# shengyangsun/LSTC_VAD

Measured on AMD Instinct MI355X. Metric: snippets/sec training step (B=64,T=32,P=16,d=2048), higher is better.
Workload: dtype f32

## Files before the change

### include/lstc_hip.h

```cpp
#ifndef LSTC_HIP_H
#define LSTC_HIP_H

#include <stdint.h>

#ifdef __cplusplus
extern "C" {
#endif

#define LSTC_VERSION 112

enum {
    LSTC_OK = 0,
    LSTC_E_NULL = -1,
    LSTC_E_SHAPE = -2,
    LSTC_E_ALIGN = -3,
    LSTC_E_UNSUPPORTED = -4,
    LSTC_E_RANGE = -5
};

enum { LSTC_F32 = 0, LSTC_BF16 = 1, LSTC_F32X3 = 2, LSTC_BF16P = 3 };

enum {
    LSTC_EPI_BIAS = 1, LSTC_EPI_RELU = 2, LSTC_EPI_DROPOUT = 4, LSTC_EPI_RESIDUAL = 8,
    LSTC_EPI_RELU_MASK = 16, LSTC_EPI_ACCUM = 32, LSTC_EPI_OUT_F32 = 64,
// ... 20 lines not shown
    const void* A;
    const void* B;
    void*       C;
    const float* bias;
    const void*  residual;
    const void*  relu_src;
} LstcGemmDesc;

int lstc_gemm(const LstcGemmDesc* d, void* stream);

int32_t lstc_gemm_splits(int32_t dtype, int32_t K, int32_t split_k);

int64_t lstc_pack3_bytes(int64_t rows, int64_t K);
int lstc_pack3(const float* src, int64_t rows, int64_t K, int64_t ld, int32_t k_major, void* dst, void* stream);

int64_t lstc_pack1_bytes(int64_t rows, int64_t K);
int lstc_pack1(const float* src, int64_t rows, int64_t K, int64_t ld, int32_t k_major, void* dst, void* stream);
typedef struct LstcPackItem {
    const float* src; int64_t rows, K, ld; int32_t k_major; void* dst;
} LstcPackItem;
int lstc_pack1_multi(const LstcPackItem* items, int32_t count, void* stream);
int lstc_colsum_pack1(const void* packed, int64_t rows, int32_t K, float* partial, int32_t n_partial, float* out,
                      int32_t accumulate, void* stream);

typedef struct LstcAttnDesc {
    int32_t N, S, H, dk, dv;
    int32_t ldq, ldk, ldv, ldo;
    int32_t dtype;
    int32_t index_ld;
    int32_t table_rows;
    float   scale;
    float   dropout_p;
    uint64_t dropout_seed;
    const void* Q; const void* K; const void* V;
    void*  O;
    float* probs;
    const float*   table;
    const int64_t* index;
    const void* dO;
    void* dQ; void* dK; void* dV;
    float* dtable;
    int32_t dtable_chunks;
    int32_t variant;
    void* dQ_pack; void* dK_pack; void* dV_pack;
    int32_t pack_cols, dQ_col0, dK_col0, dV_col0;
    void* O_pack;
// ... 129 lines not shown
```

### lstc_vad_amd/csrc/attention.hip

```cpp
#include "attention_common.h"

#ifndef ATTN_HEAD_FAST
#define ATTN_HEAD_FAST 0
#endif
#if ATTN_HEAD_FAST
#define ATTN_CHUNK ((int)blockIdx.y)
#define ATTN_HEAD ((int)blockIdx.x)
#define ATTN_GRID(chunks, H) dim3((unsigned)(H), (unsigned)(chunks))
#else
#define ATTN_CHUNK ((int)blockIdx.x)
#define ATTN_HEAD ((int)blockIdx.y)
#define ATTN_GRID(chunks, H) dim3((unsigned)(chunks), (unsigned)(H))
#endif

namespace {
using namespace lstc_attn;

constexpr int NT = 256;


__device__ __forceinline__ void load16(const float* __restrict__ p, int k0, int kdim, bool vec, float (&f)[16]) {
    if (vec && k0 + 16 <= kdim) {
        const float4* q = reinterpret_cast<const float4*>(p + k0);
#pragma unroll
// ... 759 lines not shown

extern "C" {

int lstc_attn_fwd(const LstcAttnDesc* d, void* stream) {
    AttnParams p;
    int rc = fill_params(d, p, false);
    if (rc) return rc;
    if (p.S > 128) return attn_long_fwd_launch(d, p, (hipStream_t)stream);
    if (d->O_pack) {
        const int64_t M = (int64_t)p.N * p.S;
        if (M % 256 || (p.H * p.dv) % 64 || p.dv % 32 || M * (int64_t)(p.H * p.dv) * 2 > 0x7fffffffLL) return LSTC_E_UNSUPPORTED;
        if (!aligned16(d->O_pack)) return LSTC_E_ALIGN;
        p.Op = d->O_pack;
        p.kbo = (p.H * p.dv) / 32;
    }
    hipStream_t st = (hipStream_t)stream;
    const bool bf = d->dtype == LSTC_BF16;
    const int T = (p.S + 31) / 32;
    if (d->in_pack_cols > 0) {
        if (!d->O_pack) return LSTC_E_UNSUPPORTED;
        rc = fill_packed_inputs(d, p, false);
        if (rc) return rc;
        int npw = (int)(((int64_t)p.N * p.H) / (T == 1 ? 8192 : 1024));
        if (d->variant >= 100) npw = d->variant - 100;
        npw = npw < 1 ? 1 : (npw > 16 ? 16 : npw);
        p.n_per_wg = npw;
        dim3 grid3((p.N + npw - 1) / npw, p.H);
        return attn3_fwd_launch(p, T, (int)grid3.x, st);
    }
    if (!bf && (d->variant == 3 || (d->variant == 0 && T != 2)) && d->O && T <= 3 && p.vec_qk && p.vec_v && p.dk % 32 == 0 && p.dv % 64 == 0) {
        int npw = (int)(((int64_t)p.N * p.H) / (T == 1 ? 8192 : 1024));
        npw = npw < 1 ? 1 : (npw > 16 ? 16 : npw);
        p.n_per_wg = npw;
        return attn3f_fwd_launch(p, T, (p.N + npw - 1) / npw, st);
    }
    const size_t lds = (size_t)(32 * T) * (32 * T + 1) * sizeof(float);
    dim3 grid = ATTN_GRID(p.N, p.H);
    if ((T == 1 || T == 3 || (bf && T == 2)) && p.vec_qk && p.vec_v && (p.dk % 32) == 0 && (p.dv % 32) == 0 && (d->variant == 0 || d->variant == 2)) {
        const int SP = 32 * T;
        const size_t lds2 = ((size_t)((SP * (SP + 1) + 3) & ~3) + (size_t)4 * SP * 32) * sizeof(float);
#define LSTC_FWD2(TT, BB, WW)                                                              \
    do {                                                                                   \
        static LstcDevOnce once2;                                                          \
        const int dev2_ = once2.begin();                                                   \
        if (dev2_ >= 0) { set_lds(attn_fwd2_kernel<TT, BB, WW>, 160 * 1024); once2.end(dev2_); } \
        hipLaunchKernelGGL((attn_fwd2_kernel<TT, BB, WW>), grid, 64 * WW, lds2, st, p);    \
    } while (0)
        if (!bf) { if (T == 1) LSTC_FWD2(1, false, 4); else LSTC_FWD2(3, false, 8); }
        else if (T == 1) LSTC_FWD2(1, true, 4); else if (T == 2) LSTC_FWD2(2, true, 4); else LSTC_FWD2(3, true, 8);
// ... 49 lines not shown
    p.n_per_wg = npw;
    const int chunks_ = (p.N + npw - 1) / npw;
    dim3 grid = ATTN_GRID(chunks_, p.H);
    if (p.table_partials && chunks_ != d->dtable_chunks) return LSTC_E_SHAPE;
    const bool v2 = T <= 3 && p.vec_qk && p.vec_v && (p.dk % 32) == 0 && (p.dv % 32) == 0 && d->variant != 1;
    if (d->dQ_pack || d->dK_pack || d->dV_pack) {
        const int64_t M = (int64_t)p.N * p.S;
        if (!(d->dQ_pack && d->dK_pack && d->dV_pack) || (!v2 && d->in_pack_cols <= 0) || M % 256 || (p.H * p.dk) % 64 || (p.H * p.dv) % 64 ||
            M * (int64_t)(p.H * (p.dk > p.dv ? p.dk : p.dv)) * 2 > 0x7fffffffLL) return LSTC_E_UNSUPPORTED;
        if (!aligned16(d->dQ_pack) || !aligned16(d->dK_pack) || !aligned16(d->dV_pack)) return LSTC_E_ALIGN;
        p.dQp = d->dQ_pack; p.dKp = d->dK_pack; p.dVp = d->dV_pack;
        p.kbq = p.kbk = (p.H * p.dk) / 32;
        p.kbv = (p.H * p.dv) / 32;
        if (d->pack_cols > 0) {
            if (d->pack_cols % 64 || d->dQ_col0 % 32 || d->dK_col0 % 32 || d->dV_col0 % 32 || d->dQ_col0 < 0 || d->dK_col0 < 0 || d->dV_col0 < 0 ||
                d->dQ_col0 + p.H * p.dk > d->pack_cols || d->dK_col0 + p.H * p.dk > d->pack_cols || d->dV_col0 + p.H * p.dv > d->pack_cols ||
                M * (int64_t)d->pack_cols * 2 > 0x7fffffffLL) return LSTC_E_SHAPE;
            p.kbq = p.kbk = p.kbv = d->pack_cols / 32;
            p.tq0 = d->dQ_col0 / 32; p.tk0 = d->dK_col0 / 32; p.tv0 = d->dV_col0 / 32;
        }
    }
    if (d->in_pack_cols > 0) {
        if (!p.dQp) return LSTC_E_UNSUPPORTED;
        return attn3_bwd_launch(p, T, chunks_, st);
    }
    if (v2) {
        const int SP = 32 * T, NW = T == 3 ? 8 : 4;
        const size_t lds2 = ((size_t)((2 * SP * (SP + 1) + 3) & ~3) + (size_t)4 * SP * 32 + (size_t)NW * p.table_rows) * sizeof(float);
        if (lds2 <= 160 * 1024) {
#define LSTC_BWD2(TT, BB, WW)                                                              \
    do {                                                                                   \
        static LstcDevOnce once2;                                                          \
        const int dev2_ = once2.begin();                                                   \
        if (dev2_ >= 0) { set_lds(attn_bwd2_kernel<TT, BB, WW>, 160 * 1024); once2.end(dev2_); } \
        hipLaunchKernelGGL((attn_bwd2_kernel<TT, BB, WW>), grid, 64 * WW, lds2, st, p);    \
    } while (0)
            if (T == 1) { if (bf) LSTC_BWD2(1, true, 4); else LSTC_BWD2(1, false, 4); }
            else if (T == 2) { if (bf) LSTC_BWD2(2, true, 4); else LSTC_BWD2(2, false, 4); }
            else { if (bf) LSTC_BWD2(3, true, 8); else LSTC_BWD2(3, false, 8); }
#undef LSTC_BWD2
            return lstc_launch_status();
        }
    }
    if (p.dQp) return LSTC_E_UNSUPPORTED;
#define LSTC_BWD(TT)                                                         \
    do {                                                                     \
// ... 721 lines not shown
```

### lstc_vad_amd/csrc/attention_common.h

```cpp
#pragma once
#include "lstc_common.h"

namespace lstc_attn {

struct AttnParams {
    const float *Q, *K, *V;
    float* O;
    float* probs;
    const float* table;
    const int64_t* index;
    const float* dO;
    float *dQ, *dK, *dV;
    float* dtable;
    int N, S, H, dk, dv, ldq, ldk, ldv, ldo, index_ld, table_rows;
    float scale;
    DropKey dkey;
    int has_drop;
    int vec_qk, vec_v;
    int n_per_wg;
    int table_partials;
    void *dQp, *dKp, *dVp;
    int kbq, kbk, kbv;
    int tq0, tk0, tv0;
    void* Op;
    int kbo;
    const __bf16 *Qi, *Ki, *Vi, *dOi;
    int kiq, kik, kiv, kido;
    int iq0, ik0, iv0, ido0;
    int pld;
};

typedef __bf16 attn_h8 __attribute__((ext_vector_type(8)));
typedef float attn_f2 __attribute__((ext_vector_type(2)));
typedef __bf16 attn_h2 __attribute__((ext_vector_type(2)));

__attribute__((visibility("hidden"))) int attn3_fwd_launch(const AttnParams& p, int T, int chunks, hipStream_t st);
__attribute__((visibility("hidden"))) int attn3_bwd_launch(const AttnParams& p, int T, int chunks, hipStream_t st);
__attribute__((visibility("hidden"))) int attn3f_fwd_launch(const AttnParams& p, int T, int chunks, hipStream_t st);
__attribute__((visibility("hidden"))) int attn_long_fwd_launch(const LstcAttnDesc* d, AttnParams& p, hipStream_t st);
__attribute__((visibility("hidden"))) int attn_long_bwd_launch(const LstcAttnDesc* d, AttnParams& p, hipStream_t st);

}
```

### lstc_vad_amd/csrc/attention_pk.hip

```cpp
#include "attention_common.h"

namespace {
using namespace lstc_attn;

typedef short a3_s4 __attribute__((ext_vector_type(4)));
typedef short a3_s8 __attribute__((ext_vector_type(8)));
typedef uint32_t a3_u4 __attribute__((ext_vector_type(4)));
typedef float a3_f4 __attribute__((ext_vector_type(4)));
typedef a3_s4 __attribute__((address_space(3))) * a3_lds4;

#ifndef A3_DMA_MOD
#define A3_DMA_MOD ""
#endif
__device__ __forceinline__ void a3_dma(const __bf16* tile, uint32_t voff, uint32_t lds_bytes) {
    const uint32_t lb = __builtin_amdgcn_readfirstlane(lds_bytes);
    asm volatile("s_mov_b32 m0, %2\n\ts_nop 0\n\tglobal_load_lds_dwordx4 %0, %1" A3_DMA_MOD :: "v"(voff), "s"(tile), "s"(lb) : "memory");
}
__device__ __forceinline__ uint32_t a3_row_off(uint32_t g, uint32_t kb, uint32_t lane) {
    return ((g >> 7) * kb * 4096u + (g & 127u) * 32u) * 2u + (lane & 3u) * 16u;
}
__device__ __forceinline__ attn_h8 a3_tr(const char* p0, const char* p1) {
    const a3_s4 lo = __builtin_amdgcn_ds_read_tr16_b64_v4i16((a3_lds4)p0);
    const a3_s4 hi = __builtin_amdgcn_ds_read_tr16_b64_v4i16((a3_lds4)p1);
    a3_s8 f;
// ... 8 lines not shown
    for (int g = 0; g < 4; ++g)
#pragma unroll
        for (int k = 0; k < 2; ++k) {
            attn_f2 f;
            f[0] = o[4 * g + 2 * k] * scale;
            f[1] = o[4 * g + 2 * k + 1] * scale;
            d[g][k] = __builtin_bit_cast(uint32_t, __builtin_convertvector(f, attn_h2));
        }
#pragma unroll
    for (int k = 0; k < 2; ++k) {
        const auto x = __builtin_amdgcn_permlane32_swap(d[0][k], d[2][k], false, false);
        d[0][k] = x[0]; d[2][k] = x[1];
        const auto y = __builtin_amdgcn_permlane32_swap(d[1][k], d[3][k], false, false);
        d[1][k] = y[0]; d[3][k] = y[1];
    }
    const uint32_t base = rowb + tile * 8192u;
    const a3_u4 ca = {d[0][0], d[0][1], d[2][0], d[2][1]}, cb = {d[1][0], d[1][1], d[3][0], d[3][1]};
    __builtin_amdgcn_raw_buffer_store_b128(ca, rs, valid ? base + ((((uint32_t)(2 * h2)) ^ key) << 4) : 0xFFFFFFFFu, 0, 0);
    __builtin_amdgcn_raw_buffer_store_b128(cb, rs, valid ? base + ((((uint32_t)(2 * h2 + 1)) ^ key) << 4) : 0xFFFFFFFFu, 0, 0);
}
#define A3_LDS_BARRIER() do { asm volatile("" ::: "memory"); __builtin_amdgcn_s_waitcnt(0xC07F); __builtin_amdgcn_s_barrier(); asm volatile("" ::: "memory"); } while (0)
#define A3_WAIT_VM(N) __builtin_amdgcn_s_waitcnt(((N) & 15) | (7 << 4) | (15 << 8) | (((N) >> 4) << 14))

struct A3Unit { const __bf16 *b0, *b1; uint32_t kb0, kb1; };

template <int T, int NB, typename UnitOf, typename Extra>
__device__ __forceinline__ void a3_producer(int n_begin, int n_end, int U, int S, UnitOf unit_of, Extra extra) {
    constexpr int SP = 32 * T, HALF = SP * 64, SLOT = 2 * HALF, P = 4 * T;
    static_assert(P * (NB - 2) <= 63, "vmcnt is a 6-bit counter");
    const int lane = threadIdx.x & 63;
    const int total = (n_end - n_begin) * U;
    int is_n = n_begin, is_u = 0, is_slot = 0, issued = 0;
    auto issue_next = [&]() {
        if (issued >= total) return;
        const A3Unit un = unit_of(is_u);
        const uint32_t lb = (uint32_t)(is_slot * SLOT);
#pragma unroll
        for (int pc = 0; pc < 2 * T; ++pc) {
            const uint32_t g = (uint32_t)is_n * (uint32_t)S + (uint32_t)min(16 * pc + (lane >> 2), S - 1);
            a3_dma(un.b0, a3_row_off(g, un.kb0, lane), lb + pc * 1024);
            a3_dma(un.b1, a3_row_off(g, un.kb1, lane), lb + HALF + pc * 1024);
        }
        ++issued;
        if (++is_u == U) { is_u = 0; ++is_n; }
        if (++is_slot == NB) is_slot = 0;
    };
#pragma unroll 1
    for (int k = 0; k < NB - 1; ++k) issue_next();
    int g = 0;
#pragma unroll 1
    for (int n = n_begin; n < n_end; ++n)
#pragma unroll 1
        for (int u = 0; u < U; ++u) {
            const int rem = min(NB - 2, total - 1 - g);
            if (rem >= NB - 2) A3_WAIT_VM(P * (NB - 2));
            else if (NB > 3 && rem == NB - 3) A3_WAIT_VM(P * (NB > 3 ? NB - 3 : 0));
            else if (NB > 4 && rem == NB - 4) A3_WAIT_VM(P * (NB > 4 ? NB - 4 : 0));
            else A3_WAIT_VM(0);
            __builtin_amdgcn_s_barrier();
            issue_next();
            const int nx = extra(u);
            for (int x = 0; x < nx; ++x) __builtin_amdgcn_s_barrier();
            ++g;
        }
}

template <int T, int NB>
__global__ void __launch_bounds__(64 * (T + 1)) attn_fwd3_kernel(const AttnParams p) {
    const DropKey dkn = drop_key_now(p.dkey);
    constexpr int SP = 32 * T, HALF = SP * 64, SLOT = 2 * HALF;
    extern __shared__ __attribute__((aligned(16))) float sm[];
    const char* ring = reinterpret_cast<const char*>(sm);
    const int h = (int)(blockIdx.x % (unsigned)p.H), chunk = (int)(blockIdx.x / (unsigned)p.H), S = p.S;
    const int lane = threadIdx.x & 63, wave = __builtin_amdgcn_readfirstlane(threadIdx.x >> 6);
    const int l31 = lane & 31, h2 = lane >> 5;
    const int n_begin = chunk * p.n_per_wg, n_end = min(p.N, n_begin + p.n_per_wg);
    const int nq = p.dk >> 5, nvp = p.dv >> 6, U = nq + nvp;
    if (wave == T) {
        const int tq = p.iq0 + ((h * p.dk) >> 5), tk = p.ik0 + ((h * p.dk) >> 5), tv = p.iv0 + ((h * p.dv) >> 5);
        a3_producer<T, NB>(n_begin, n_end, U, S,
            [&](int u) -> A3Unit {
                A3Unit un;
                if (u < nq) {
                    un.b0 = p.Qi + (size_t)(tq + u) * 4096; un.kb0 = (uint32_t)p.kiq;
                    un.b1 = p.Ki + (size_t)(tk + u) * 4096; un.kb1 = (uint32_t)p.kik;
                } else {
                    un.b0 = p.Vi + (size_t)(tv + 2 * (u - nq)) * 4096; un.kb0 = un.kb1 = (uint32_t)p.kiv;
                    un.b1 = un.b0 + 4096;
                }
                return un;
            },
            [](int) { return 0; });
        return;
    }
    const int i = 32 * wave + l31;
    const bool has_bias = p.index_ld > 0 && S > 1;
    const __amdgpu_buffer_rsrc_t r_index = __builtin_amdgcn_make_buffer_rsrc(const_cast<int64_t*>(p.index), 0,
        has_bias ? (S - 1) * p.index_ld * 8 : 0, 0x00020000);
    const __amdgpu_buffer_rsrc_t r_table = __builtin_amdgcn_make_buffer_rsrc(const_cast<float*>(p.table), 0,
        has_bias ? (p.table_rows > 0 ? p.table_rows * p.H * 4 : 0x7fffffff) : 0, 0x00020000);
    float biasr[T][16];
#pragma unroll
    for (int t = 0; t < T; ++t)
#pragma unroll
        for (int r = 0; r < 16; ++r) {
            const int j = 32 * t + 8 * (r >> 2) + 4 * h2 + (r & 3);
            const bool pair = i >= 1 && j >= 1 && i < S && j < S;
            const uint32_t ix = __builtin_amdgcn_raw_buffer_load_b32(r_index, pair ? (uint32_t)((i - 1) * p.index_ld + (j - 1)) * 8u : 0xFFFFFFFFu, 0, 0);
            const float b = __builtin_bit_cast(float, __builtin_amdgcn_raw_buffer_load_b32(r_table, ((ix * (uint32_t)p.H + (uint32_t)h) * 4u) | (pair ? 0u : 0xFFFFFFFFu), 0, 0));
            biasr[t][r] = b + (j < S ? 0.f : -INFINITY);
        }
    const __amdgpu_buffer_rsrc_t r_Op = __builtin_amdgcn_make_buffer_rsrc(p.Op, 0, (int)0x7fffffff, 0x00020000);
    const int q4 = (lane >> 2) & 3, p4 = lane & 3, gg = (lane >> 4) & 1;
    int cslot = 0;
    floatx16 acc[T];
    attn_h8 pf[T][2];
#pragma unroll 1
    for (int n = n_begin; n < n_end; ++n) {
        const uint32_t r0 = (uint32_t)n * (uint32_t)S;
        const uint32_t keyq = ((r0 + (uint32_t)i) >> 2) & 3u, keyk = ((r0 + (uint32_t)l31) >> 2) & 3u;
        const int offq0 = i * 64 + (int)(((0 + h2) ^ keyq) << 4), offq1 = i * 64 + (int)(((2 + h2) ^ keyq) << 4);
        const int offk0 = l31 * 64 + (int)(((0 + h2) ^ keyk) << 4), offk1 = l31 * 64 + (int)(((2 + h2) ^ keyk) << 4);
        int troff[2];
#pragma unroll
        for (int rd = 0; rd < 2; ++rd) {
            const uint32_t row = (uint32_t)(4 * h2 + 8 * rd + q4);
            troff[rd] = (int)(row * 64u + ((((uint32_t)(2 * gg + (p4 >> 1))) ^ (((r0 + row) >> 2) & 3u)) << 4) + 8u * (uint32_t)(p4 & 1));
        }
        const uint32_t orow = a3_row_off(r0 + (uint32_t)i, (uint32_t)p.kbo, 0);
#pragma unroll 1
        for (int u = 0; u < U; ++u) {
            A3_LDS_BARRIER();
            const char* slot = ring + cslot * SLOT;
            if (u < nq) {
                if (u == 0) {
#pragma unroll
                    for (int t = 0; t < T; ++t)
#pragma unroll
                        for (int r = 0; r < 16; ++r) acc[t][r] = 0.f;
                }
                const attn_h8 fq0 = a3_row(slot + offq0), fq1 = a3_row(slot + offq1);
#pragma unroll
                for (int t = 0; t < T; ++t) {
                    const attn_h8 fk0 = a3_row(slot + HALF + t * 2048 + offk0), fk1 = a3_row(slot + HALF + t * 2048 + offk1);
                    acc[t] = __builtin_amdgcn_mfma_f32_32x32x16_bf16(fk0, fq0, acc[t], 0, 0, 0);
                    acc[t] = __builtin_amdgcn_mfma_f32_32x32x16_bf16(fk1, fq1, acc[t], 0, 0, 0);
                }
                if (u == nq - 1) {
                    float m = -INFINITY;
#pragma unroll
                    for (int t = 0; t < T; ++t)
#pragma unroll
                        for (int r = 0; r < 16; ++r) {
                            const float x = acc[t][r] * p.scale + biasr[t][r];
                            acc[t][r] = x;
                            m = fmaxf(m, x);
                        }
                    m = fmaxf(m, __shfl_xor(m, 32, 64));
                    float sum = 0.f;
#pragma unroll
                    for (int t = 0; t < T; ++t)
#pragma unroll
                        for (int r = 0; r < 16; ++r) {
                            const float e = expf(acc[t][r] - m);
                            acc[t][r] = e;
                            sum += e;
                        }
// ... 17 lines not shown
                                float v = pv[e];
                                if (p.has_drop) v = drop_keep(flat_i + (uint32_t)(j0 + e), dkn) ? v * dkn.scale : 0.f;
                                acc[t][4 * g4 + e] = v;
                            }
                        }
#pragma unroll
                        for (int s2 = 0; s2 < 2; ++s2)
#pragma unroll
                            for (int e = 0; e < 8; ++e) pf[t][s2][e] = (__bf16)acc[t][8 * s2 + e];
                    }
                }
            } else {
                const int ct = 2 * (u - nq);
#pragma unroll
                for (int hf = 0; hf < 2; ++hf) {
                    const char* Vs = slot + hf * HALF;
                    floatx16 o[1];
#pragma unroll
                    for (int r = 0; r < 16; ++r) o[0][r] = 0.f;
#pragma unroll
                    for (int t = 0; t < T; ++t)
#pragma unroll
                        for (int s2 = 0; s2 < 2; ++s2) {
                            const attn_h8 fv = a3_tr(Vs + t * 2048 + s2 * 1024 + troff[0], Vs + t * 2048 + s2 * 1024 + troff[1]);
                            o[0] = __builtin_amdgcn_mfma_f32_32x32x16_bf16(fv, pf[t][s2], o[0], 0, 0, 0);
                        }
                    a3_store_tile(o[0], 1.f, r_Op, orow, keyq, i < S, (uint32_t)(((h * p.dv) >> 5) + ct + hf), h2);
                }
            }
            if (++cslot == NB) cslot = 0;
        }
    }
}

template <int T, int NB>
__global__ void __launch_bounds__(64 * (T + 1)) attn_bwd3_kernel(const AttnParams p) {
    const DropKey dkn = drop_key_now(p.dkey);
    constexpr int SP = 32 * T, HALF = SP * 64, SLOT = 2 * HALF;
    constexpr int ILD = 72, IMG = SP * ILD;
    extern __shared__ __attribute__((aligned(16))) float sm[];
    char* ring = reinterpret_cast<char*>(sm);
    char* img = ring + NB * SLOT;
    float* tacc = reinterpret_cast<float*>(img + IMG);
    const int h = (int)(blockIdx.x % (unsigned)p.H), chunk = (int)(blockIdx.x / (unsigned)p.H), S = p.S;
    const int lane = threadIdx.x & 63, wave = __builtin_amdgcn_readfirstlane(threadIdx.x >> 6);
    const int l31 = lane & 31, h2 = lane >> 5;
    const int n_begin = chunk * p.n_per_wg, n_end = min(p.N, n_begin + p.n_per_wg);
    const int nv = p.dv >> 5, nq2 = p.dk >> 6, nv2 = p.dv >> 6;
    const int u_c1 = nv, u_c2 = nv + nq2, u_c3 = nv + nq2 + nv2, U = nv + 2 * nq2 + nv2;
    const bool has_bias = p.index_ld > 0 && p.dtable != nullptr;
    if (has_bias)
        for (int x = threadIdx.x; x < T * p.table_rows; x += 64 * (T + 1)) tacc[x] = 0.f;
    __syncthreads();
    if (wave == T) {
        const int tq = p.iq0 + ((h * p.dk) >> 5), tk = p.ik0 + ((h * p.dk) >> 5), tv = p.iv0 + ((h * p.dv) >> 5), tdo = p.ido0 + ((h * p.dv) >> 5);
        a3_producer<T, NB>(n_begin, n_end, U, S,
            [&](int u) -> A3Unit {
                A3Unit un;
                if (u < u_c1) {
                    un.b0 = p.dOi + (size_t)(tdo + u) * 4096; un.kb0 = (uint32_t)p.kido;
                    un.b1 = p.Vi + (size_t)(tv + u) * 4096; un.kb1 = (uint32_t)p.kiv;
                } else if (u < u_c2) {
                    un.b0 = p.Ki + (size_t)(tk + 2 * (u - u_c1)) * 4096; un.kb0 = un.kb1 = (uint32_t)p.kik; un.b1 = un.b0 + 4096;
                } else if (u < u_c3) {
                    un.b0 = p.dOi + (size_t)(tdo + 2 * (u - u_c2)) * 4096; un.kb0 = un.kb1 = (uint32_t)p.kido; un.b1 = un.b0 + 4096;
                } else {
                    un.b0 = p.Qi + (size_t)(tq + 2 * (u - u_c3)) * 4096; un.kb0 = un.kb1 = (uint32_t)p.kiq; un.b1 = un.b0 + 4096;
                }
                return un;
            },
            [&](int u) { return u == u_c1 - 1 ? 4 * T : 0; });
    } else {
    const int i = 32 * wave + l31;
    float* const tw = tacc + wave * p.table_rows;
    const __amdgpu_buffer_rsrc_t r_index = __builtin_amdgcn_make_buffer_rsrc(const_cast<int64_t*>(p.index), 0,
        (has_bias && S > 1) ? (S - 1) * p.index_ld * 8 : 0, 0x00020000);
    uint32_t idxp[T][8];
#pragma unroll
    for (int t = 0; t < T; ++t)
#pragma unroll
        for (int r2 = 0; r2 < 8; ++r2) {
            uint32_t w2 = 0;
#pragma unroll
            for (int e = 0; e < 2; ++e) {
                const int r = 2 * r2 + e;
                const int j = 32 * t + 8 * (r >> 2) + 4 * h2 + (r & 3);
                const bool pair = has_bias && i >= 1 && j >= 1 && i < S && j < S;
                const uint32_t v = __builtin_amdgcn_raw_buffer_load_b32(r_index, pair ? (uint32_t)((i - 1) * p.index_ld + (j - 1)) * 8u : 0xFFFFFFFFu, 0, 0)
                                   | (pair ? 0u : 0xFFFFu);
                w2 |= (v & 0xFFFFu) << (16 * e);
            }
            idxp[t][r2] = w2;
        }
    const __amdgpu_buffer_rsrc_t r_dQ = __builtin_amdgcn_make_buffer_rsrc(p.dQp, 0, (int)0x7fffffff, 0x00020000);
    const __amdgpu_buffer_rsrc_t r_dK = __builtin_amdgcn_make_buffer_rsrc(p.dKp, 0, (int)0x7fffffff, 0x00020000);
    const __amdgpu_buffer_rsrc_t r_dV = __builtin_amdgcn_make_buffer_rsrc(p.dVp, 0, (int)0x7fffffff, 0x00020000);
    const int q4 = (lane >> 2) & 3, p4 = lane & 3, gg = (lane >> 4) & 1;
    char* const img_w = img + i * ILD + 8 * h2;
    const char* const img_r = img + (8 * h2 + q4) * ILD + 32 * gg + 8 * p4;
    int cslot = 0;
    floatx16 acc[T];
    float prr[T][16];
    attn_h8 dAf[T][2], PdTf[T][2], dATf[T][2];
    float dsum[T][16];
#pragma unroll
    for (int t = 0; t < T; ++t)
#pragma unroll
        for (int r = 0; r < 16; ++r) dsum[t][r] = 0.f;
#pragma unroll 1
    for (int n = n_begin; n < n_end; ++n) {
        const uint32_t r0 = (uint32_t)n * (uint32_t)S;
        const uint32_t keyq = ((r0 + (uint32_t)i) >> 2) & 3u, keyk = ((r0 + (uint32_t)l31) >> 2) & 3u;
        const int offq0 = i * 64 + (int)(((0 + h2) ^ keyq) << 4), offq1 = i * 64 + (int)(((2 + h2) ^ keyq) << 4);
        const int offk0 = l31 * 64 + (int)(((0 + h2) ^ keyk) << 4), offk1 = l31 * 64 + (int)(((2 + h2) ^ keyk) << 4);
        int troff[2], trnat[2];
#pragma unroll
        for (int rd = 0; rd < 2; ++rd) {
            const uint32_t row = (uint32_t)(4 * h2 + 8 * rd + q4), rown = (uint32_t)(8 * h2 + 4 * rd + q4);
            troff[rd] = (int)(row * 64u + ((((uint32_t)(2 * gg + (p4 >> 1))) ^ (((r0 + row) >> 2) & 3u)) << 4) + 8u * (uint32_t)(p4 & 1));
            trnat[rd] = (int)(rown * 64u + ((((uint32_t)(2 * gg + (p4 >> 1))) ^ (((r0 + rown) >> 2) & 3u)) << 4) + 8u * (uint32_t)(p4 & 1));
        }
#pragma unroll 1
        for (int u = 0; u < U; ++u) {
            A3_LDS_BARRIER();
            const char* slot = ring + cslot * SLOT;
            if (u < u_c1) {
                if (u == 0) {
                    const float* pr_item = p.probs + ((size_t)n * p.H + h) * S * p.pld;
#pragma unroll
                    for (int t = 0; t < T; ++t)
#pragma unroll
                        for (int g4 = 0; g4 < 4; ++g4) {
                            const int j0 = 32 * t + 8 * g4 + 4 * h2;
                            const bool ok = i < S && j0 < p.pld;
                            const a3_u4 v = *reinterpret_cast<const a3_u4*>(pr_item + (ok ? i * p.pld + j0 : 0));
                            const uint32_t mask = ok ? 0xFFFFFFFFu : 0u;
#pragma unroll
                            for (int e = 0; e < 4; ++e) prr[t][4 * g4 + e] = __builtin_bit_cast(float, v[e] & mask);
                        }
#pragma unroll
                    for (int t = 0; t < T; ++t)
#pragma unroll
                        for (int r = 0; r < 16; ++r) acc[t][r] = 0.f;
                }
                const attn_h8 fo0 = a3_row(slot + offq0), fo1 = a3_row(slot + offq1);
#pragma unroll
                for (int t = 0; t < T; ++t) {
                    const attn_h8 fv0 = a3_row(slot + HALF + t * 2048 + offk0), fv1 = a3_row(slot + HALF + t * 2048 + offk1);
                    acc[t] = __builtin_amdgcn_mfma_f32_32x32x16_bf16(fv0, fo0, acc[t], 0, 0, 0);
                    acc[t] = __builtin_amdgcn_mfma_f32_32x32x16_bf16(fv1, fo1, acc[t], 0, 0, 0);
                }
                if (u == u_c1 - 1) {
                    typedef __bf16 h4v __attribute__((ext_vector_type(4)));
                    const uint32_t flat_i = ((uint32_t)n * p.H + h) * (uint32_t)(S * S) + (uint32_t)(i * S);
                    float rs = 0.f;
                    h4v pdp[T][4];
#pragma unroll
                    for (int t = 0; t < T; ++t)
#pragma unroll
                        for (int g4 = 0; g4 < 4; ++g4) {
#pragma unroll
                            for (int e = 0; e < 4; ++e) {
                                const int r = 4 * g4 + e;
                                const int j = 32 * t + 8 * g4 + 4 * h2 + e;
                                const float keep = p.has_drop ? (drop_keep(flat_i + (uint32_t)j, dkn) ? dkn.scale : 0.f) : 1.f;
                                const float dpk = acc[t][r] * keep;
                                rs += dpk * prr[t][r];
                                acc[t][r] = dpk;
                                pdp[t][g4][e] = (__bf16)(prr[t][r] * keep);
                            }
                        }
// ... 39 lines not shown
#pragma unroll
                            for (int ti = 0; ti < T; ++ti)
#pragma unroll
                                for (int s2 = 0; s2 < 2; ++s2)
                                    dATf[ti][s2] = a3_tr(img_r + (32 * ti + 16 * s2) * ILD, img_r + (32 * ti + 16 * s2 + 4) * ILD);
                        }
                        A3_LDS_BARRIER();
                    }
                }
            } else {
                const int ph = u < u_c2 ? 0 : (u < u_c3 ? 1 : 2);
                const int ct = 2 * (u - (ph == 0 ? u_c1 : (ph == 1 ? u_c2 : u_c3)));
#pragma unroll
                for (int hf = 0; hf < 2; ++hf) {
                    const char* Bs = slot + hf * HALF;
                    floatx16 o[1];
#pragma unroll
                    for (int r = 0; r < 16; ++r) o[0][r] = 0.f;
                    if (ph == 0) {
#pragma unroll
                        for (int t = 0; t < T; ++t)
#pragma unroll
                            for (int s2 = 0; s2 < 2; ++s2) {
                                const attn_h8 fb = a3_tr(Bs + t * 2048 + s2 * 1024 + troff[0], Bs + t * 2048 + s2 * 1024 + troff[1]);
                                o[0] = __builtin_amdgcn_mfma_f32_32x32x16_bf16(fb, dAf[t][s2], o[0], 0, 0, 0);
                            }
                        a3_store_tile(o[0], p.scale, r_dQ, a3_row_off(r0 + (uint32_t)i, (uint32_t)p.kbq, 0), keyq, i < S, (uint32_t)(p.tq0 + ((h * p.dk) >> 5) + ct + hf), h2);
                    } else if (ph == 1) {
#pragma unroll
                        for (int t = 0; t < T; ++t)
#pragma unroll
                            for (int s2 = 0; s2 < 2; ++s2) {
                                const attn_h8 fb = a3_tr(Bs + t * 2048 + s2 * 1024 + trnat[0], Bs + t * 2048 + s2 * 1024 + trnat[1]);
                                o[0] = __builtin_amdgcn_mfma_f32_32x32x16_bf16(fb, PdTf[t][s2], o[0], 0, 0, 0);
                            }
                        a3_store_tile(o[0], 1.f, r_dV, a3_row_off(r0 + (uint32_t)i, (uint32_t)p.kbv, 0), keyq, i < S, (uint32_t)(p.tv0 + ((h * p.dv) >> 5) + ct + hf), h2);
                    } else {
#pragma unroll
                        for (int t = 0; t < T; ++t)
#pragma unroll
                            for (int s2 = 0; s2 < 2; ++s2) {
                                const attn_h8 fb = a3_tr(Bs + t * 2048 + s2 * 1024 + trnat[0], Bs + t * 2048 + s2 * 1024 + trnat[1]);
                                o[0] = __builtin_amdgcn_mfma_f32_32x32x16_bf16(fb, dATf[t][s2], o[0], 0, 0, 0);
                            }
                        a3_store_tile(o[0], p.scale, r_dK, a3_row_off(r0 + (uint32_t)i, (uint32_t)p.kbk, 0), keyq, i < S, (uint32_t)(p.tk0 + ((h * p.dk) >> 5) + ct + hf), h2);
                    }
                }
            }
            if (++cslot == NB) cslot = 0;
        }
    }
    if (has_bias) {
#pragma unroll
        for (int t = 0; t < T; ++t)
#pragma unroll
            for (int r = 0; r < 16; ++r) {
                const uint32_t ix = (idxp[t][r >> 1] >> (16 * (r & 1))) & 0xFFFFu;
                if (ix != 0xFFFFu) atomicAdd(&tw[ix], dsum[t][r]);
            }
    }
    }
    if (has_bias) {
        __syncthreads();
        for (int x = threadIdx.x; x < p.table_rows; x += 64 * (T + 1)) {
            float v = tacc[x];
#pragma unroll
            for (int w = 1; w < T; ++w) v += tacc[w * p.table_rows + x];
            if (p.table_partials) p.dtable[((size_t)chunk * p.table_rows + x) * p.H + h] = v;
            else atomicAdd(&p.dtable[(size_t)x * p.H + h], v);
        }
    }
}

struct A3UnitF { const float *b0, *b1; uint32_t ld0, ld1; };

// ... 190 lines not shown
                        for (int g4 = 0; g4 < 4; ++g4) {
                            a3_f4 v;
#pragma unroll
                            for (int e = 0; e < 4; ++e) v[e] = o[4 * g4 + e];
                            *reinterpret_cast<a3_f4*>(o_row + 32 * (ct + hf) + 8 * g4 + 4 * h2) = v;
                        }
                    }
                }
            }
            if (++cslot == NB) cslot = 0;
        }
    }
}

template <typename Kern>
void set_lds(Kern k, size_t lds) {
    (void)hipFuncSetAttribute(reinterpret_cast<const void*>(k), hipFuncAttributeMaxDynamicSharedMemorySize, (int)lds);
}

}

namespace lstc_attn {

int attn3_fwd_launch(const AttnParams& p, int T, int chunks, hipStream_t st) {
#define LSTC_FWD3(TT, NBB)                                                                 \
    do {                                                                                   \
        static LstcDevOnce once3;                                                          \
        const int dev3_ = once3.begin();                                                   \
        if (dev3_ >= 0) { set_lds(attn_fwd3_kernel<TT, NBB>, 160 * 1024); once3.end(dev3_); } \
        hipLaunchKernelGGL((attn_fwd3_kernel<TT, NBB>), dim3((unsigned)chunks * (unsigned)p.H), 64 * (TT + 1), \
                           (size_t)NBB * 2 * (32 * TT) * 64, st, p);                       \
    } while (0)
    if (T == 1) LSTC_FWD3(1, 6); else if (T == 2) LSTC_FWD3(2, 9); else if (T == 3) LSTC_FWD3(3, 6); else return LSTC_E_RANGE;
#undef LSTC_FWD3
    return lstc_launch_status();
}

int attn3f_fwd_launch(const AttnParams& p, int T, int chunks, hipStream_t st) {
#define LSTC_FWD3F(TT, NBB)                                                                \
    do {                                                                                   \
        static LstcDevOnce once3;                                                          \
        const int dev3_ = once3.begin();                                                   \
        if (dev3_ >= 0) { set_lds(attn_fwd3f_kernel<TT, NBB>, 160 * 1024); once3.end(dev3_); } \
        hipLaunchKernelGGL((attn_fwd3f_kernel<TT, NBB>), dim3((unsigned)chunks * (unsigned)p.H), 64 * (TT + 1), \
                           (size_t)NBB * 2 * (32 * TT) * 128, st, p);                      \
    } while (0)
    if (T == 1) LSTC_FWD3F(1, 3); else if (T == 2) LSTC_FWD3F(2, 3); else if (T == 3) LSTC_FWD3F(3, 3); else return LSTC_E_RANGE;
#undef LSTC_FWD3F
    return lstc_launch_status();
}

int attn3_bwd_launch(const AttnParams& p, int T, int chunks, hipStream_t st) {
#define LSTC_BWD3(TT, NBB)                                                                 \
    do {                                                                                   \
        const size_t lds3 = (size_t)NBB * 2 * (32 * TT) * 64 + (size_t)(32 * TT) * 72 + (size_t)TT * p.table_rows * sizeof(float); \
        if (lds3 > 160 * 1024) return LSTC_E_RANGE;                                        \
        static LstcDevOnce once3;                                                          \
        const int dev3_ = once3.begin();                                                   \
        if (dev3_ >= 0) { set_lds(attn_bwd3_kernel<TT, NBB>, 160 * 1024); once3.end(dev3_); } \
        hipLaunchKernelGGL((attn_bwd3_kernel<TT, NBB>), dim3((unsigned)chunks * (unsigned)p.H), 64 * (TT + 1), lds3, st, p); \
    } while (0)
    if (T == 1) LSTC_BWD3(1, 9); else if (T == 2) LSTC_BWD3(2, 8); else if (T == 3) LSTC_BWD3(3, 5); else return LSTC_E_RANGE;
#undef LSTC_BWD3
    return lstc_launch_status();
}

}
```

Before: 22870.

## Size attention LDS ring to actual sequence rows and pick depth at runtime

The packed bf16 attention forward and backward kernels now size their LDS staging ring to the real sequence length, S rounded up to 4 rows, instead of the full 32*T padded tile. The ring depth is chosen on the host to balance pipeline depth against workgroups per CU, and launch bounds now request multiple waves per EU. The producer loads only the rows it needs, the last key/value tile maps rows with a clamped index, and the vmcnt wait becomes a runtime switch. The backward kernel also defers the index/bias gather until after the main loop to cut register pressure. The cost is extra address arithmetic, a switch-based wait, and possible reads of stale rows in partially filled tiles.

```diff
diff --git a/include/lstc_hip.h b/include/lstc_hip.h
--- a/include/lstc_hip.h
+++ b/include/lstc_hip.h
@@ -66,6 +66,8 @@
 int lstc_pack1_multi(const LstcPackItem* items, int32_t count, void* stream);
 int lstc_colsum_pack1(const void* packed, int64_t rows, int32_t K, float* partial, int32_t n_partial, float* out,
                       int32_t accumulate, void* stream);
+
+#define LSTC_ATTN_VARIANT_RING32 (1 << 30)
 
 typedef struct LstcAttnDesc {
     int32_t N, S, H, dk, dv;
diff --git a/lstc_vad_amd/csrc/attention.hip b/lstc_vad_amd/csrc/attention.hip
--- a/lstc_vad_amd/csrc/attention.hip
+++ b/lstc_vad_amd/csrc/attention.hip
@@ -805,9 +805,11 @@
         rc = fill_packed_inputs(d, p, false);
         if (rc) return rc;
         int npw = (int)(((int64_t)p.N * p.H) / (T == 1 ? 8192 : 1024));
-        if (d->variant >= 100) npw = d->variant - 100;
+        const int hook = d->variant & ~LSTC_ATTN_VARIANT_RING32;
+        if (hook >= 100) npw = hook - 100;
         npw = npw < 1 ? 1 : (npw > 16 ? 16 : npw);
         p.n_per_wg = npw;
+        p.ring_wide = (d->variant & LSTC_ATTN_VARIANT_RING32) != 0;
         dim3 grid3((p.N + npw - 1) / npw, p.H);
         return attn3_fwd_launch(p, T, (int)grid3.x, st);
     }
@@ -903,6 +905,7 @@
     }
     if (d->in_pack_cols > 0) {
         if (!p.dQp) return LSTC_E_UNSUPPORTED;
+        p.ring_wide = (d->variant & LSTC_ATTN_VARIANT_RING32) != 0;
         return attn3_bwd_launch(p, T, chunks_, st);
     }
     if (v2) {
diff --git a/lstc_vad_amd/csrc/attention_common.h b/lstc_vad_amd/csrc/attention_common.h
--- a/lstc_vad_amd/csrc/attention_common.h
+++ b/lstc_vad_amd/csrc/attention_common.h
@@ -28,6 +28,7 @@
     int kiq, kik, kiv, kido;
     int iq0, ik0, iv0, ido0;
     int pld;
+    int ring_wide, ring_rows, ring_nb;
 };
 
 typedef __bf16 attn_h8 __attribute__((ext_vector_type(8)));
diff --git a/lstc_vad_amd/csrc/attention_pk.hip b/lstc_vad_amd/csrc/attention_pk.hip
--- a/lstc_vad_amd/csrc/attention_pk.hip
+++ b/lstc_vad_amd/csrc/attention_pk.hip
@@ -1,4 +1,5 @@
 #include "attention_common.h"
+#include <cstdlib>
 
 namespace {
 using namespace lstc_attn;
@@ -54,12 +55,23 @@
 #define A3_LDS_BARRIER() do { asm volatile("" ::: "memory"); __builtin_amdgcn_s_waitcnt(0xC07F); __builtin_amdgcn_s_barrier(); asm volatile("" ::: "memory"); } while (0)
 #define A3_WAIT_VM(N) __builtin_amdgcn_s_waitcnt(((N) & 15) | (7 << 4) | (15 << 8) | (((N) >> 4) << 14))
 
+__device__ __forceinline__ void a3_wait_vm(int n) {
+    switch (n) {
+#define A3_W(N) case N: A3_WAIT_VM(N); break;
+        A3_W(2) A3_W(4) A3_W(6) A3_W(8) A3_W(10) A3_W(12) A3_W(14) A3_W(16) A3_W(18) A3_W(20) A3_W(22) A3_W(24) A3_W(26) A3_W(28) A3_W(30) A3_W(32)
+        A3_W(34) A3_W(36) A3_W(38) A3_W(40) A3_W(42) A3_W(44) A3_W(46) A3_W(48) A3_W(50) A3_W(52) A3_W(54) A3_W(56) A3_W(58) A3_W(60) A3_W(62)
+#undef A3_W
+        default: A3_WAIT_VM(0); break;
+    }
+}
+
 struct A3Unit { const __bf16 *b0, *b1; uint32_t kb0, kb1; };
 
-template <int T, int NB, typename UnitOf, typename Extra>
-__device__ __forceinline__ void a3_producer(int n_begin, int n_end, int U, int S, UnitOf unit_of, Extra extra) {
-    constexpr int SP = 32 * T, HALF = SP * 64, SLOT = 2 * HALF, P = 4 * T;
-    static_assert(P * (NB - 2) <= 63, "vmcnt is a 6-bit counter");
+__device__ __forceinline__ int a3_tile_row(int row, int SR) { return row < SR ? row : SR - 4 + (row & 3); }
+
+template <int T, typename UnitOf, typename Extra>
+__device__ __forceinline__ void a3_producer(int n_begin, int n_end, int U, int S, int SR, int NB, UnitOf unit_of, Extra extra) {
+    const int HALF = SR * 64, SLOT = 2 * HALF, PH = (SR + 15) >> 4, P = 2 * PH;
     const int lane = threadIdx.x & 63;
     const int total = (n_end - n_begin) * U;
     int is_n = n_begin, is_u = 0, is_slot = 0, issued = 0;
@@ -69,9 +81,13 @@
         const uint32_t lb = (uint32_t)(is_slot * SLOT);
 #pragma unroll
         for (int pc = 0; pc < 2 * T; ++pc) {
-            const uint32_t g = (uint32_t)is_n * (uint32_t)S + (uint32_t)min(16 * pc + (lane >> 2), S - 1);
-            a3_dma(un.b0, a3_row_off(g, un.kb0, lane), lb + pc * 1024);
-            a3_dma(un.b1, a3_row_off(g, un.kb1, lane), lb + HALF + pc * 1024);
+            if (pc >= PH) break;
+            const int row = 16 * pc + (lane >> 2);
+            if (row < SR) {
+                const uint32_t g = (uint32_t)is_n * (uint32_t)S + (uint32_t)min(row, S - 1);
+                a3_dma(un.b0, a3_row_off(g, un.kb0, lane), lb + pc * 1024);
+                a3_dma(un.b1, a3_row_off(g, un.kb1, lane), lb + HALF + pc * 1024);
+            }
         }
         ++issued;
         if (++is_u == U) { is_u = 0; ++is_n; }
@@ -84,11 +100,7 @@
     for (int n = n_begin; n < n_end; ++n)
 #pragma unroll 1
         for (int u = 0; u < U; ++u) {
-            const int rem = min(NB - 2, total - 1 - g);
-            if (rem >= NB - 2) A3_WAIT_VM(P * (NB - 2));
-            else if (NB > 3 && rem == NB - 3) A3_WAIT_VM(P * (NB > 3 ? NB - 3 : 0));
-            else if (NB > 4 && rem == NB - 4) A3_WAIT_VM(P * (NB > 4 ? NB - 4 : 0));
-            else A3_WAIT_VM(0);
+            a3_wait_vm(P * min(NB - 2, total - 1 - g));
             __builtin_amdgcn_s_barrier();
             issue_next();
             const int nx = extra(u);
@@ -97,10 +109,10 @@
         }
 }
 
-template <int T, int NB>
-__global__ void __launch_bounds__(64 * (T + 1)) attn_fwd3_kernel(const AttnParams p) {
+template <int T>
+__global__ void __launch_bounds__(64 * (T + 1), T == 2 ? 3 : (T == 3 ? 2 : 1)) attn_fwd3_kernel(const AttnParams p) {
     const DropKey dkn = drop_key_now(p.dkey);
-    constexpr int SP = 32 * T, HALF = SP * 64, SLOT = 2 * HALF;
+    const int SR = p.ring_rows, NB = p.ring_nb, HALF = SR * 64, SLOT = 2 * HALF;
     extern __shared__ __attribute__((aligned(16))) float sm[];
     const char* ring = reinterpret_cast<const char*>(sm);
     const int h = (int)(blockIdx.x % (unsigned)p.H), chunk = (int)(blockIdx.x / (unsigned)p.H), S = p.S;
@@ -110,7 +122,7 @@
     const int nq = p.dk >> 5, nvp = p.dv >> 6, U = nq + nvp;
     if (wave == T) {
         const int tq = p.iq0 + ((h * p.dk) >> 5), tk = p.ik0 + ((h * p.dk) >> 5), tv = p.iv0 + ((h * p.dv) >> 5);
-        a3_producer<T, NB>(n_begin, n_end, U, S,
+        a3_producer<T>(n_begin, n_end, U, S, SR, NB,
             [&](int u) -> A3Unit {
                 A3Unit un;
                 if (u < nq) {
@@ -126,6 +138,7 @@
         return;
     }
     const int i = 32 * wave + l31;
+    const int iq = a3_tile_row(i, SR), kL = a3_tile_row(32 * (T - 1) + l31, SR);
     const bool has_bias = p.index_ld > 0 && S > 1;
     const __amdgpu_buffer_rsrc_t r_index = __builtin_amdgcn_make_buffer_rsrc(const_cast<int64_t*>(p.index), 0,
         has_bias ? (S - 1) * p.index_ld * 8 : 0, 0x00020000);
@@ -151,13 +164,20 @@
     for (int n = n_begin; n < n_end; ++n) {
         const uint32_t r0 = (uint32_t)n * (uint32_t)S;
         const uint32_t keyq = ((r0 + (uint32_t)i) >> 2) & 3u, keyk = ((r0 + (uint32_t)l31) >> 2) & 3u;
-        const int offq0 = i * 64 + (int)(((0 + h2) ^ keyq) << 4), offq1 = i * 64 + (int)(((2 + h2) ^ keyq) << 4);
+        const int offq0 = iq * 64 + (int)(((0 + h2) ^ keyq) << 4), offq1 = iq * 64 + (int)(((2 + h2) ^ keyq) << 4);
         const int offk0 = l31 * 64 + (int)(((0 + h2) ^ keyk) << 4), offk1 = l31 * 64 + (int)(((2 + h2) ^ keyk) << 4);
-        int troff[2];
+        const int offkL0 = kL * 64 + (int)(((0 + h2) ^ keyk) << 4), offkL1 = kL * 64 + (int)(((2 + h2) ^ keyk) << 4);
+        int troff[2], troffL[2][2];
 #pragma unroll
         for (int rd = 0; rd < 2; ++rd) {
             const uint32_t row = (uint32_t)(4 * h2 + 8 * rd + q4);
-            troff[rd] = (int)(row * 64u + ((((uint32_t)(2 * gg + (p4 >> 1))) ^ (((r0 + row) >> 2) & 3u)) << 4) + 8u * (uint32_t)(p4 & 1));
+            const uint32_t ck = (uint32_t)(2 * gg + (p4 >> 1)), b8 = 8u * (uint32_t)(p4 & 1);
+            troff[rd] = (int)(row * 64u + ((ck ^ (((r0 + row) >> 2) & 3u)) << 4) + b8);
+#pragma unroll
+            for (int s2 = 0; s2 < 2; ++s2) {
+                const uint32_t rl = (uint32_t)(32 * (T - 1) + 16 * s2) + row;
+                troffL[s2][rd] = (int)((uint32_t)a3_tile_row((int)rl, SR) * 64u + ((ck ^ (((r0 + rl) >> 2) & 3u)) << 4) + b8);
+            }
         }
         const uint32_t orow = a3_row_off(r0 + (uint32_t)i, (uint32_t)p.kbo, 0);
 #pragma unroll 1
@@ -174,7 +194,8 @@
                 const attn_h8 fq0 = a3_row(slot + offq0), fq1 = a3_row(slot + offq1);
 #pragma unroll
                 for (int t = 0; t < T; ++t) {
-                    const attn_h8 fk0 = a3_row(slot + HALF + t * 2048 + offk0), fk1 = a3_row(slot + HALF + t * 2048 + offk1);
+                    const attn_h8 fk0 = a3_row(slot + HALF + (t < T - 1 ? t * 2048 + offk0 : offkL0));
+                    const attn_h8 fk1 = a3_row(slot + HALF + (t < T - 1 ? t * 2048 + offk1 : offkL1));
                     acc[t] = __builtin_amdgcn_mfma_f32_32x32x16_bf16(fk0, fq0, acc[t], 0, 0, 0);
                     acc[t] = __builtin_amdgcn_mfma_f32_32x32x16_bf16(fk1, fq1, acc[t], 0, 0, 0);
                 }
@@ -238,7 +259,8 @@
                     for (int t = 0; t < T; ++t)
 #pragma unroll
                         for (int s2 = 0; s2 < 2; ++s2) {
-                            const attn_h8 fv = a3_tr(Vs + t * 2048 + s2 * 1024 + troff[0], Vs + t * 2048 + s2 * 1024 + troff[1]);
+                            const attn_h8 fv = t < T - 1 ? a3_tr(Vs + t * 2048 + s2 * 1024 + troff[0], Vs + t * 2048 + s2 * 1024 + troff[1])
+                                                         : a3_tr(Vs + troffL[s2][0], Vs + troffL[s2][1]);
                             o[0] = __builtin_amdgcn_mfma_f32_32x32x16_bf16(fv, pf[t][s2], o[0], 0, 0, 0);
                         }
                     a3_store_tile(o[0], 1.f, r_Op, orow, keyq, i < S, (uint32_t)(((h * p.dv) >> 5) + ct + hf), h2);
@@ -249,10 +271,11 @@
     }
 }
 
-template <int T, int NB>
-__global__ void __launch_bounds__(64 * (T + 1)) attn_bwd3_kernel(const AttnParams p) {
+template <int T>
+__global__ void __launch_bounds__(64 * (T + 1), T == 2 ? 2 : 1) attn_bwd3_kernel(const AttnParams p) {
     const DropKey dkn = drop_key_now(p.dkey);
-    constexpr int SP = 32 * T, HALF = SP * 64, SLOT = 2 * HALF;
+    constexpr int SP = 32 * T;
+    const int SR = p.ring_rows, NB = p.ring_nb, HALF = SR * 64, SLOT = 2 * HALF;
     constexpr int ILD = 72, IMG = SP * ILD;
     extern __shared__ __attribute__((aligned(16))) float sm[];
     char* ring = reinterpret_cast<char*>(sm);
@@ -270,7 +293,7 @@
     __syncthreads();
     if (wave == T) {
         const int tq = p.iq0 + ((h * p.dk) >> 5), tk = p.ik0 + ((h * p.dk) >> 5), tv = p.iv0 + ((h * p.dv) >> 5), tdo = p.ido0 + ((h * p.dv) >> 5);
-        a3_producer<T, NB>(n_begin, n_end, U, S,
+        a3_producer<T>(n_begin, n_end, U, S, SR, NB,
             [&](int u) -> A3Unit {
                 A3Unit un;
                 if (u < u_c1) {
@@ -288,26 +311,8 @@
             [&](int u) { return u == u_c1 - 1 ? 4 * T : 0; });
     } else {
     const int i = 32 * wave + l31;
+    const int iq = a3_tile_row(i, SR), kL = a3_tile_row(32 * (T - 1) + l31, SR);
     float* const tw = tacc + wave * p.table_rows;
-    const __amdgpu_buffer_rsrc_t r_index = __builtin_amdgcn_make_buffer_rsrc(const_cast<int64_t*>(p.index), 0,
-        (has_bias && S > 1) ? (S - 1) * p.index_ld * 8 : 0, 0x00020000);
-    uint32_t idxp[T][8];
-#pragma unroll
-    for (int t = 0; t < T; ++t)
-#pragma unroll
-        for (int r2 = 0; r2 < 8; ++r2) {
-            uint32_t w2 = 0;
-#pragma unroll
-            for (int e = 0; e < 2; ++e) {
-                const int r = 2 * r2 + e;
-                const int j = 32 * t + 8 * (r >> 2) + 4 * h2 + (r & 3);
-                const bool pair = has_bias && i >= 1 && j >= 1 && i < S && j < S;
-                const uint32_t v = __builtin_amdgcn_raw_buffer_load_b32(r_index, pair ? (uint32_t)((i - 1) * p.index_ld + (j - 1)) * 8u : 0xFFFFFFFFu, 0, 0)
-                                   | (pair ? 0u : 0xFFFFu);
-                w2 |= (v & 0xFFFFu) << (16 * e);
-            }
-            idxp[t][r2] = w2;
-        }
     const __amdgpu_buffer_rsrc_t r_dQ = __builtin_amdgcn_make_buffer_rsrc(p.dQp, 0, (int)0x7fffffff, 0x00020000);
     const __amdgpu_buffer_rsrc_t r_dK = __builtin_amdgcn_make_buffer_rsrc(p.dKp, 0, (int)0x7fffffff, 0x00020000);
     const __amdgpu_buffer_rsrc_t r_dV = __builtin_amdgcn_make_buffer_rsrc(p.dVp, 0, (int)0x7fffffff, 0x00020000);
@@ -327,14 +332,22 @@
     for (int n = n_begin; n < n_end; ++n) {
         const uint32_t r0 = (uint32_t)n * (uint32_t)S;
         const uint32_t keyq = ((r0 + (uint32_t)i) >> 2) & 3u, keyk = ((r0 + (uint32_t)l31) >> 2) & 3u;
-        const int offq0 = i * 64 + (int)(((0 + h2) ^ keyq) << 4), offq1 = i * 64 + (int)(((2 + h2) ^ keyq) << 4);
+        const int offq0 = iq * 64 + (int)(((0 + h2) ^ keyq) << 4), offq1 = iq * 64 + (int)(((2 + h2) ^ keyq) << 4);
         const int offk0 = l31 * 64 + (int)(((0 + h2) ^ keyk) << 4), offk1 = l31 * 64 + (int)(((2 + h2) ^ keyk) << 4);
-        int troff[2], trnat[2];
+        const int offkL0 = kL * 64 + (int)(((0 + h2) ^ keyk) << 4), offkL1 = kL * 64 + (int)(((2 + h2) ^ keyk) << 4);
+        int troff[2], trnat[2], troffL[2][2], trnatL[2][2];
 #pragma unroll
         for (int rd = 0; rd < 2; ++rd) {
             const uint32_t row = (uint32_t)(4 * h2 + 8 * rd + q4), rown = (uint32_t)(8 * h2 + 4 * rd + q4);
-            troff[rd] = (int)(row * 64u + ((((uint32_t)(2 * gg + (p4 >> 1))) ^ (((r0 + row) >> 2) & 3u)) << 4) + 8u * (uint32_t)(p4 & 1));
-            trnat[rd] = (int)(rown * 64u + ((((uint32_t)(2 * gg + (p4 >> 1))) ^ (((r0 + rown) >> 2) & 3u)) << 4) + 8u * (uint32_t)(p4 & 1));
+            const uint32_t ck = (uint32_t)(2 * gg + (p4 >> 1)), b8 = 8u * (uint32_t)(p4 & 1);
+            troff[rd] = (int)(row * 64u + ((ck ^ (((r0 + row) >> 2) & 3u)) << 4) + b8);
+            trnat[rd] = (int)(rown * 64u + ((ck ^ (((r0 + rown) >> 2) & 3u)) << 4) + b8);
+#pragma unroll
+            for (int s2 = 0; s2 < 2; ++s2) {
+                const uint32_t rl = (uint32_t)(32 * (T - 1) + 16 * s2) + row, rln = (uint32_t)(32 * (T - 1) + 16 * s2) + rown;
+                troffL[s2][rd] = (int)((uint32_t)a3_tile_row((int)rl, SR) * 64u + ((ck ^ (((r0 + rl) >> 2) & 3u)) << 4) + b8);
+                trnatL[s2][rd] = (int)((uint32_t)a3_tile_row((int)rln, SR) * 64u + ((ck ^ (((r0 + rln) >> 2) & 3u)) << 4) + b8);
+            }
         }
 #pragma unroll 1
         for (int u = 0; u < U; ++u) {
@@ -362,7 +375,8 @@
                 const attn_h8 fo0 = a3_row(slot + offq0), fo1 = a3_row(slot + offq1);
 #pragma unroll
                 for (int t = 0; t < T; ++t) {
-                    const attn_h8 fv0 = a3_row(slot + HALF + t * 2048 + offk0), fv1 = a3_row(slot + HALF + t * 2048 + offk1);
+                    const attn_h8 fv0 = a3_row(slot + HALF + (t < T - 1 ? t * 2048 + offk0 : offkL0));
+                    const attn_h8 fv1 = a3_row(slot + HALF + (t < T - 1 ? t * 2048 + offk1 : offkL1));
                     acc[t] = __builtin_amdgcn_mfma_f32_32x32x16_bf16(fv0, fo0, acc[t], 0, 0, 0);
                     acc[t] = __builtin_amdgcn_mfma_f32_32x32x16_bf16(fv1, fo1, acc[t], 0, 0, 0);
                 }
@@ -448,7 +462,8 @@
                         for (int t = 0; t < T; ++t)
 #pragma unroll
                             for (int s2 = 0; s2 < 2; ++s2) {
-                                const attn_h8 fb = a3_tr(Bs + t * 2048 + s2 * 1024 + troff[0], Bs + t * 2048 + s2 * 1024 + troff[1]);
+                                const attn_h8 fb = t < T - 1 ? a3_tr(Bs + t * 2048 + s2 * 1024 + troff[0], Bs + t * 2048 + s2 * 1024 + troff[1])
+                                                             : a3_tr(Bs + troffL[s2][0], Bs + troffL[s2][1]);
                                 o[0] = __builtin_amdgcn_mfma_f32_32x32x16_bf16(fb, dAf[t][s2], o[0], 0, 0, 0);
                             }
                         a3_store_tile(o[0], p.scale, r_dQ, a3_row_off(r0 + (uint32_t)i, (uint32_t)p.kbq, 0), keyq, i < S, (uint32_t)(p.tq0 + ((h * p.dk) >> 5) + ct + hf), h2);
@@ -457,7 +472,8 @@
                         for (int t = 0; t < T; ++t)
 #pragma unroll
                             for (int s2 = 0; s2 < 2; ++s2) {
-                                const attn_h8 fb = a3_tr(Bs + t * 2048 + s2 * 1024 + trnat[0], Bs + t * 2048 + s2 * 1024 + trnat[1]);
+                                const attn_h8 fb = t < T - 1 ? a3_tr(Bs + t * 2048 + s2 * 1024 + trnat[0], Bs + t * 2048 + s2 * 1024 + trnat[1])
+                                                             : a3_tr(Bs + trnatL[s2][0], Bs + trnatL[s2][1]);
                                 o[0] = __builtin_amdgcn_mfma_f32_32x32x16_bf16(fb, PdTf[t][s2], o[0], 0, 0, 0);
                             }
                         a3_store_tile(o[0], 1.f, r_dV, a3_row_off(r0 + (uint32_t)i, (uint32_t)p.kbv, 0), keyq, i < S, (uint32_t)(p.tv0 + ((h * p.dv) >> 5) + ct + hf), h2);
@@ -466,7 +482,8 @@
                         for (int t = 0; t < T; ++t)
 #pragma unroll
                             for (int s2 = 0; s2 < 2; ++s2) {
-                                const attn_h8 fb = a3_tr(Bs + t * 2048 + s2 * 1024 + trnat[0], Bs + t * 2048 + s2 * 1024 + trnat[1]);
+                                const attn_h8 fb = t < T - 1 ? a3_tr(Bs + t * 2048 + s2 * 1024 + trnat[0], Bs + t * 2048 + s2 * 1024 + trnat[1])
+                                                             : a3_tr(Bs + trnatL[s2][0], Bs + trnatL[s2][1]);
                                 o[0] = __builtin_amdgcn_mfma_f32_32x32x16_bf16(fb, dATf[t][s2], o[0], 0, 0, 0);
                             }
                         a3_store_tile(o[0], p.scale, r_dK, a3_row_off(r0 + (uint32_t)i, (uint32_t)p.kbk, 0), keyq, i < S, (uint32_t)(p.tk0 + ((h * p.dk) >> 5) + ct + hf), h2);
@@ -477,6 +494,25 @@
         }
     }
     if (has_bias) {
+        const __amdgpu_buffer_rsrc_t r_index = __builtin_amdgcn_make_buffer_rsrc(const_cast<int64_t*>(p.index), 0,
+            (has_bias && S > 1) ? (S - 1) * p.index_ld * 8 : 0, 0x00020000);
+        uint32_t idxp[T][8];
+    #pragma unroll
+        for (int t = 0; t < T; ++t)
+    #pragma unroll
+            for (int r2 = 0; r2 < 8; ++r2) {
+                uint32_t w2 = 0;
+    #pragma unroll
+                for (int e = 0; e < 2; ++e) {
+                    const int r = 2 * r2 + e;
+                    const int j = 32 * t + 8 * (r >> 2) + 4 * h2 + (r & 3);
+                    const bool pair = has_bias && i >= 1 && j >= 1 && i < S && j < S;
+                    const uint32_t v = __builtin_amdgcn_raw_buffer_load_b32(r_index, pair ? (uint32_t)((i - 1) * p.index_ld + (j - 1)) * 8u : 0xFFFFFFFFu, 0, 0)
+                                       | (pair ? 0u : 0xFFFFu);
+                    w2 |= (v & 0xFFFFu) << (16 * e);
+                }
+                idxp[t][r2] = w2;
+            }
 #pragma unroll
         for (int t = 0; t < T; ++t)
 #pragma unroll
@@ -713,16 +749,51 @@
 
 namespace lstc_attn {
 
-int attn3_fwd_launch(const AttnParams& p, int T, int chunks, hipStream_t st) {
-#define LSTC_FWD3(TT, NBB)                                                                 \
+bool a3_ring(AttnParams& p, int T, bool wide, int nb_wide, int max_wpc, size_t extra, size_t* lds) {
+    const int SR = wide ? 32 * T : (p.S + 3) / 4 * 4;
+    const size_t slot = (size_t)2 * SR * 64;
+    int nb = nb_wide;
+    if (!wide) {
+        const int nb_vm = 2 + 63 / (2 * ((SR + 15) / 16));
+        int best = 0, nb_of[9] = {0};
+        for (int w = 1; w <= max_wpc && w <= 8; ++w) {
+            const size_t budget = (size_t)(160 * 1024) / w;
+            int n = budget > extra ? (int)((budget - extra) / slot) : 0;
+            n = n > nb_vm ? nb_vm : n;
+            nb_of[w] = n;
+            if (n >= 3 && (n - 1) * w > best) best = (n - 1) * w;
+        }
+        nb = 0;
+        for (int w = 1; w <= max_wpc && w <= 8; ++w)
+            if (nb_of[w] >= 3 && 10 * (nb_of[w] - 1) * w >= 9 * best) nb = nb_of[w];
+    }
+#ifdef LSTC_TUNING
+    if (const char* e = getenv("LSTC_A3_NB")) {
+        const int n = atoi(e);
+        if (n >= 3 && 2 * ((SR + 15) / 16) * (n - 2) <= 63) nb = n;
+    }
+#endif
+    *lds = (size_t)nb * slot + extra;
+    if (nb < 3 || *lds > 160 * 1024) return false;
+    p.ring_rows = SR;
+    p.ring_nb = nb;
+    return true;
+}
+
+int attn3_fwd_launch(const AttnParams& p_, int T, int chunks, hipStream_t st) {
+    AttnParams p = p_;
+    size_t lds3 = 0;
+    static const int nb_wide[3] = {6, 9, 6}, max_wpc[3] = {8, 3, 2};
+    if (T < 1 || T > 3) return LSTC_E_RANGE;
+    if (!a3_ring(p, T, p.ring_wide != 0, nb_wide[T - 1], max_wpc[T - 1], 0, &lds3)) return LSTC_E_RANGE;
+#define LSTC_FWD3(TT)                                                                      \
     do {                                                                                   \
         static LstcDevOnce once3;                                                          \
         const int dev3_ = once3.begin();                                                   \
-        if (dev3_ >= 0) { set_lds(attn_fwd3_kernel<TT, NBB>, 160 * 1024); once3.end(dev3_); } \
-        hipLaunchKernelGGL((attn_fwd3_kernel<TT, NBB>), dim3((unsigned)chunks * (unsigned)p.H), 64 * (TT + 1), \
-                           (size_t)NBB * 2 * (32 * TT) * 64, st, p);                       \
+        if (dev3_ >= 0) { set_lds(attn_fwd3_kernel<TT>, 160 * 1024); once3.end(dev3_); }   \
+        hipLaunchKernelGGL((attn_fwd3_kernel<TT>), dim3((unsigned)chunks * (unsigned)p.H), 64 * (TT + 1), lds3, st, p); \
     } while (0)
-    if (T == 1) LSTC_FWD3(1, 6); else if (T == 2) LSTC_FWD3(2, 9); else if (T == 3) LSTC_FWD3(3, 6); else return LSTC_E_RANGE;
+    if (T == 1) LSTC_FWD3(1); else if (T == 2) LSTC_FWD3(2); else LSTC_FWD3(3);
 #undef LSTC_FWD3
     return lstc_launch_status();
 }
@@ -741,17 +812,21 @@
     return lstc_launch_status();
 }
 
-int attn3_bwd_launch(const AttnParams& p, int T, int chunks, hipStream_t st) {
-#define LSTC_BWD3(TT, NBB)                                                                 \
+int attn3_bwd_launch(const AttnParams& p_, int T, int chunks, hipStream_t st) {
+    AttnParams p = p_;
+    size_t lds3 = 0;
+    static const int nb_wide[3] = {9, 8, 5}, max_wpc[3] = {4, 2, 1};
+    if (T < 1 || T > 3) return LSTC_E_RANGE;
+    const size_t extra = (size_t)(32 * T) * 72 + (size_t)T * p.table_rows * sizeof(float);
+    if (!a3_ring(p, T, p.ring_wide != 0, nb_wide[T - 1], max_wpc[T - 1], extra, &lds3)) return LSTC_E_RANGE;
+#define LSTC_BWD3(TT)                                                                      \
     do {                                                                                   \
-        const size_t lds3 = (size_t)NBB * 2 * (32 * TT) * 64 + (size_t)(32 * TT) * 72 + (size_t)TT * p.table_rows * sizeof(float); \
-        if (lds3 > 160 * 1024) return LSTC_E_RANGE;                                        \
         static LstcDevOnce once3;                                                          \
         const int dev3_ = once3.begin();                                                   \
-        if (dev3_ >= 0) { set_lds(attn_bwd3_kernel<TT, NBB>, 160 * 1024); once3.end(dev3_); } \
-        hipLaunchKernelGGL((attn_bwd3_kernel<TT, NBB>), dim3((unsigned)chunks * (unsigned)p.H), 64 * (TT + 1), lds3, st, p); \
+        if (dev3_ >= 0) { set_lds(attn_bwd3_kernel<TT>, 160 * 1024); once3.end(dev3_); }   \
+        hipLaunchKernelGGL((attn_bwd3_kernel<TT>), dim3((unsigned)chunks * (unsigned)p.H), 64 * (TT + 1), lds3, st, p); \
     } while (0)
-    if (T == 1) LSTC_BWD3(1, 9); else if (T == 2) LSTC_BWD3(2, 8); else if (T == 3) LSTC_BWD3(3, 5); else return LSTC_E_RANGE;
+    if (T == 1) LSTC_BWD3(1); else if (T == 2) LSTC_BWD3(2); else LSTC_BWD3(3);
 #undef LSTC_BWD3
     return lstc_launch_status();
 }
```

New measurement: 22800 (median of 2 runs). No clear change (-0.3%).
